# vwxyzjn/cleanrl

Hardware: AMD Instinct MI355X
Metric: env-steps/sec (SPS) PPO Breakout num_envs=1024 @1/2/4/8 MI355X; GAE HBM GB/s (higher is better)
Workload: dtype f32

## Files before the change

cleanrl_amd/build.py:

```python
from __future__ import annotations

import os
import subprocess
import sys
from concurrent.futures import ThreadPoolExecutor

CSRC = os.path.join(os.path.dirname(os.path.abspath(__file__)), "csrc")
LIB = os.path.join(CSRC, "libmi355ppo.so")
SOURCES = ["api.hip", "gae.hip", "distributions.hip", "loss.hip", "obs.hip", "optim.hip", "conv.hip", "convw.hip", "conv1q.hip", "conv1p.hip", "gemmz.hip", "gemmg.hip", "gemmh.hip", "convr.hip", "convrb.hip", "convrs.hip", "convu.hip", "fcw.hip", "heads.hip", "mlp.hip", "synth_env.hip", "dpcomm.hip", "lstm.hip", "trxl_attn.hip", "impala.hip", "pqn.hip", "pqn_lstm.hip", "offpolicy.hip", "sac.hip", "dqn.hip", "dqn_atari.hip", "rainbow.hip", "rainbow_twins.hip", "sac_atari.hip", "sac_atari_twins.hip", "qdagger.hip", "rnd.hip", "ppg.hip", "ppg_twins.hip", "host_twins.hip"]
HEADERS = ["common.h", "catrow.h", "ppo_rows.h", "lstm_rows.h", "trxl_rows.h", "impala_rows.h", "pqn_rows.h", "pqn_lstm_rows.h", "offpolicy_rows.h", "offpolicy_wg.h", "qhead_wg.h", "sac_rows.h", "dqn_rows.h", "dqn_atari_rows.h", "rainbow_rows.h", "sac_atari_rows.h", "qdagger_rows.h", "rnd_rows.h", "ppg_rows.h", "bf16split.h", "f16split.h", "convr_geom.h", "convrb_geom.h", "convrs_geom.h", os.path.join("..", "..", "include", "mi355ppo.h")]
HIPCC = os.environ.get("HIPCC", "/opt/rocm/bin/hipcc")
FLAGS = ["--offload-arch=gfx950", "-O3", "-std=c++20", "-ffp-contract=off", "-fPIC", "-fvisibility=hidden", "-Wall", "-Wno-unused-function"]
EXTRA_FLAGS = {"conv.hip": ["-mllvm", "-pragma-unroll-threshold=1000000"], "gemmz.hip": ["-fno-slp-vectorize"], "gemmg.hip": ["-fno-slp-vectorize"], "gemmh.hip": ["-fno-slp-vectorize", "-mllvm", "-pragma-unroll-threshold=1000000"], "convr.hip": ["-fno-slp-vectorize", "-mllvm", "-pragma-unroll-threshold=1000000"], "convrb.hip": ["-fno-slp-vectorize", "-mllvm", "-pragma-unroll-threshold=1000000"], "convrs.hip": ["-fno-slp-vectorize", "-mllvm", "-pragma-unroll-threshold=1000000"], "convu.hip": ["-fno-slp-vectorize", "-mllvm", "-pragma-unroll-threshold=1000000"], "fcw.hip": ["-fno-slp-vectorize"], "convw.hip": ["-fno-slp-vectorize"], "lstm.hip": ["-fno-slp-vectorize"], "pqn_lstm.hip": ["-fno-slp-vectorize"]}


def _stale(target: str, deps: list[str]) -> bool:
    if not os.path.exists(target):
        return True
    t = os.path.getmtime(target)
    return any(os.path.getmtime(d) > t for d in deps)


def _run(cmd: list[str]) -> None:
    r = subprocess.run(cmd, cwd=CSRC, capture_output=True, text=True)
    if r.returncode != 0:
        raise RuntimeError("command failed: %s\n%s\n%s" % (" ".join(cmd), r.stdout, r.stderr))


def build(force: bool = False, verbose: bool = True) -> str:
    hdrs = [os.path.join(CSRC, h) for h in HEADERS]
    objs, jobs = [], []
    for src in SOURCES:
        obj = os.path.join(CSRC, src.replace(".hip", ".o"))
        objs.append(obj)
        if force or _stale(obj, [os.path.join(CSRC, src)] + hdrs):
            jobs.append([HIPCC] + FLAGS + EXTRA_FLAGS.get(src, []) + ["-c", src, "-o", obj])
    if jobs:
        if verbose:
            print(f"[cleanrl_amd.build] compiling {len(jobs)} HIP source(s) for gfx950", file=sys.stderr)
        with ThreadPoolExecutor(max_workers=min(len(jobs), os.cpu_count() or 1)) as ex:
            list(ex.map(_run, jobs))
    if force or jobs or _stale(LIB, objs):
        _run([HIPCC, "--offload-arch=gfx950", "-shared", "-o", LIB] + objs)
        if verbose:
            print(f"[cleanrl_amd.build] linked {LIB}", file=sys.stderr)
    return LIB


def build_tools(verbose: bool = True) -> str:
    root = os.path.dirname(os.path.dirname(CSRC))
    src = os.path.join(root, "tools", "conv_traffic.cpp")
    exe = os.path.join(root, "tools", "conv_traffic")
    if _stale(exe, [src, LIB, os.path.join(root, "include", "mi355ppo.h")]):
        _run([HIPCC, "--offload-arch=gfx950", "-O2", "-I" + os.path.join(root, "include"), src, "-o", exe, "-L" + CSRC,
              "-lmi355ppo", "-Wl,-rpath,$ORIGIN/../cleanrl_amd/csrc"])
        if verbose:
            print(f"[cleanrl_amd.build] built {exe}", file=sys.stderr)
    fsrc, fexe = os.path.join(root, "tools", "mfma_floor.cpp"), os.path.join(root, "tools", "mfma_floor")
    if os.path.exists(fsrc) and _stale(fexe, [fsrc]):
        _run([HIPCC, "--offload-arch=gfx950", "-O3", fsrc, "-o", fexe])
        if verbose:
            print(f"[cleanrl_amd.build] built {fexe}", file=sys.stderr)
    psrc, pexe = os.path.join(root, "tools", "hbm_probe.cpp"), os.path.join(root, "tools", "hbm_probe")
    if os.path.exists(psrc) and _stale(pexe, [psrc]):
        _run([HIPCC, "--offload-arch=gfx950", "-O3", psrc, "-o", pexe])
        if verbose:
            print(f"[cleanrl_amd.build] built {pexe}", file=sys.stderr)
    dsrc, dexe = os.path.join(root, "tools", "mfma_denorm.cpp"), os.path.join(root, "tools", "mfma_denorm")
    if os.path.exists(dsrc) and _stale(dexe, [dsrc]):
        _run([HIPCC, "--offload-arch=gfx950", "-O2", "-Wno-unused-result", dsrc, "-o", dexe])
        if verbose:
            print(f"[cleanrl_amd.build] built {dexe}", file=sys.stderr)
    return exe


if __name__ == "__main__":
    build(force="--force" in sys.argv)
    build_tools()
```

cleanrl_amd/csrc/common.h:

```cpp
#pragma once
#include <hip/hip_runtime.h>
#include <stdint.h>
#include <stdio.h>
#include <stdarg.h>
#include <stdlib.h>

#include "../../include/mi355ppo.h"

#define MI355_WAVE 64
#ifndef MI355_AUX_WGRAD_LD
#define MI355_AUX_WGRAD_LD 2
#endif
#ifndef MI355_AUX_STREAM_LD
#define MI355_AUX_STREAM_LD 0
#endif
#ifndef MI355_AUX_STREAM_ST
#define MI355_AUX_STREAM_ST 0
#endif
#define MI355_HD __host__ __device__ __forceinline__

namespace mi355ppo {

void set_error(const char* fmt, ...);

int conv1p_launch(const unsigned char* src, const int64_t* inds, const float* dz, float* part_w, float* part_b, int images, int grid,
                  hipStream_t s, const unsigned* dz_amax, float* partial_scale);
bool convw_applies(int64_t images, int layer, bool f16 = false);
int convw_parts(int64_t images, int layer);
int convw_launch(const float* src, const float* dz, float* part_w, float* part_b, int64_t images, int layer, int* nparts, hipStream_t s,
                 const unsigned* dz_amax = nullptr, const unsigned* src_amax = nullptr);

bool convr_on(long long images, long long min_images);
int convr_fwd3(const char* fn, const float* src, unsigned src_bytes, const void* pack, const float* bias, float* dst, unsigned dst_bytes, unsigned* bits,
               long long images, const unsigned* src_amax, unsigned* dst_amax, hipStream_t st);
int convr_fwd2(const char* fn, const float* src, unsigned src_bytes, const void* pack, const float* bias, float* dst, unsigned dst_bytes, unsigned* bits,
               long long images, const unsigned* src_amax, unsigned* dst_amax, hipStream_t st);
int convr_dgrad3(const char* fn, const float* dz, unsigned dz_bytes, const void* pack, const unsigned* bits, float* dsrc, unsigned dsrc_bytes,
                 long long images, const unsigned* dz_amax, unsigned* dsrc_amax, hipStream_t st);
int convr_dgrad2(const char* fn, const float* dz, unsigned dz_bytes, const void* pack, const unsigned* bits, float* dsrc, unsigned dsrc_bytes,
                 long long images, const unsigned* dz_amax, unsigned* dsrc_amax, hipStream_t st);
#ifndef MI355_RING_DMA
#define MI355_RING_DMA 1
#endif
#ifndef MI355_RB_MIN_IMAGES
#define MI355_RB_MIN_IMAGES 3072
#endif
bool convrb_takes(long long images);
int convrb_dgrad2(const char* fn, const float* dz, unsigned dz_bytes, const void* pack, const unsigned* bits, float* dsrc, unsigned dsrc_bytes,
                  long long images, const unsigned* dz_amax, unsigned* dsrc_amax, hipStream_t st);
#ifndef MI355_RS_MIN_IMAGES
#define MI355_RS_MIN_IMAGES 512
#endif
bool convrs_takes(long long images);
int convrs_fwd2(const char* fn, const float* src, unsigned src_bytes, const void* pack, const float* bias, float* dst, unsigned dst_bytes, unsigned* bits,
                long long images, const unsigned* src_amax, unsigned* dst_amax, hipStream_t st);
int convu_max_parts();
bool convu_takes(int64_t images, int layer);
int convu_launch(const float* src, const float* dz, float* part_w, float* part_b, int64_t images, int layer, int* nparts, hipStream_t s,
                 const unsigned* dz_amax, const unsigned* src_amax);
int convu1_launch(const unsigned char* frames, const int64_t* inds, const float* dz, float* part_w, float* part_b, int64_t images, int* nparts,
                  hipStream_t s, const unsigned* dz_amax);
bool gemmg_on(long long rows, long long min_rows);
int gemmg_launch(const char* fn, int epi, const float* A, int lda, const void* pack, const float* bias, const unsigned* bits, float* C, int M, int N,
                 int K, const unsigned* a_amax, unsigned* c_amax, hipStream_t s);
bool gemmh_takes(int M, int N, int K, int lddz);
int gemmh_slabs();
int gemmh_launch(const float* dz, int lddz, const float* a, float* part, int M, int N, int K, const unsigned* dz_amax, const unsigned* a_amax, hipStream_t s);
int z_fc_raw_launch(const char* fn, const float* a, int lda, const void* pack, int M, int N, int K, void* ws, size_t ws_bytes, int* splits,
                    hipStream_t stream, const unsigned* a_amax = nullptr);

inline hipStream_t as_stream(void* s) { return reinterpret_cast<hipStream_t>(s); }

inline int bf16_term_pairs() {
    static const int n = [] {
        const char* e = getenv("MI355PPO_BF16_PAIRS");
        return (e && e[0] == '9') ? 9 : 6;
    }();
    return n;
}

inline bool kernel_switch(const char* name, long long size, long long default_min) {
    const char* e = getenv(name);
    if (!e || !e[0]) return size >= default_min;
    if (e[0] == '0' && !e[1]) return false;
    if (e[0] == 'm' && e[1] == 'i' && e[2] == 'n' && e[3] == ':') return size >= atoll(e + 4);
    return size >= default_min;
}

inline bool aligned(const void* p, size_t a) { return (reinterpret_cast<uintptr_t>(p) % a) == 0; }

inline int check_launch(const char* what) {
    hipError_t e = hipGetLastError();
    if (e != hipSuccess) {
        set_error("%s: %s", what, hipGetErrorString(e));
        return MI355PPO_EHIP;
    }
    return MI355PPO_OK;
}

#define MI355_REQUIRE(cond, code, ...)          \
    do {                                        \
        if (!(cond)) {                          \
            ::mi355ppo::set_error(__VA_ARGS__); \
            return (code);                      \
        }                                       \
    } while (0)

#ifdef __HIPCC__

MI355_HD uint32_t mulhi_u32(uint32_t a, uint32_t b) {
#if defined(__HIP_DEVICE_COMPILE__)
    return __umulhi(a, b);
#else
    return (uint32_t)(((uint64_t)a * (uint64_t)b) >> 32);
#endif
}

struct Philox {
    uint32_t k0, k1;
    MI355_HD Philox(uint64_t seed) : k0((uint32_t)seed), k1((uint32_t)(seed >> 32)) {}
    MI355_HD uint4 operator()(uint64_t ctr_lo, uint64_t ctr_hi) const {
        uint32_t c0 = (uint32_t)ctr_lo, c1 = (uint32_t)(ctr_lo >> 32), c2 = (uint32_t)ctr_hi, c3 = (uint32_t)(ctr_hi >> 32);
        uint32_t a = k0, b = k1;
#pragma unroll
        for (int r = 0; r < 10; ++r) {
            const uint32_t hi0 = mulhi_u32(0xD2511F53u, c0), lo0 = 0xD2511F53u * c0;
            const uint32_t hi1 = mulhi_u32(0xCD9E8D57u, c2), lo1 = 0xCD9E8D57u * c2;
            const uint32_t n0 = hi1 ^ c1 ^ a, n1 = lo1, n2 = hi0 ^ c3 ^ b, n3 = lo0;
            c0 = n0; c1 = n1; c2 = n2; c3 = n3;
            a += 0x9E3779B9u; b += 0xBB67AE85u;
        }
        return make_uint4(c0, c1, c2, c3);
    }
};

MI355_HD float u32_to_unit_open(uint32_t x) {
    return ((float)(x >> 9) + 0.5f) * (1.0f / 8388608.0f);
}


__device__ __forceinline__ float wave_sum(float v) {
#pragma unroll
    for (int off = 32; off > 0; off >>= 1) v += __shfl_xor(v, off, MI355_WAVE);
    return v;
}
__device__ __forceinline__ double wave_sum(double v) {
#pragma unroll
    for (int off = 32; off > 0; off >>= 1) v += __shfl_xor(v, off, MI355_WAVE);
    return v;
}

template <int NWAVES>
__device__ __forceinline__ double block_sum(double v, double* lds) {
    v = wave_sum(v);
    const int lane = threadIdx.x & 63, wave = threadIdx.x >> 6;
    if (lane == 0) lds[wave] = v;
    __syncthreads();
    double r = 0.0;
    if (threadIdx.x == 0) {
#pragma unroll
        for (int w = 0; w < NWAVES; ++w) r += lds[w];
    }
    __syncthreads();
    return r;
}

#endif
}
```

cleanrl_amd/csrc/gemmz.hip:

```cpp
#include "common.h"
#include "conv1q_pack.h"
#include "bf16split.h"
#include "f16split.h"
#include <type_traits>

#pragma clang fp contract(off)

namespace mi355ppo {

typedef float z_f32x16 __attribute__((ext_vector_type(16)));

__device__ __forceinline__ int z_writelane(int w, unsigned x, int l) {
    asm("s_nop 1\n\tv_writelane_b32 %0, %1, %2" : "+v"(w) : "s"(x), "i"(l));
    return w;
}

enum { Z_BIAS_RELU = 0, Z_MASK = 1, Z_MASK_CLS4 = 2, Z_MASKB = 3, Z_MASKB_CLS4 = 4, Z_BIAS_RELU_BITS = 5, Z_RAW = 6 };

__device__ __forceinline__ float z_keep_where(float x, unsigned lo, unsigned hi) {
    const unsigned long long m = ((unsigned long long)hi << 32) | lo;
    float r;
    asm("s_nop 1\n\tv_cndmask_b32_e64 %0, 0, %1, %2" : "=v"(r) : "v"(x), "s"(m));
    return r;
}
// ... 1001 lines not shown
    ZArgs za = zargs(a, (long long)M * lda * 4, lda, pack, bias, nullptr, h, (long long)M * N * 4, N, M, N, K);
    za.a_amax = a_amax; za.c_amax = h_amax;
    if (a_amax && fc_g_takes(M, N, K, false)) {
        rc = gemmg_launch(fn, 0, a, lda, pack, bias, nullptr, h, M, N, K, a_amax, h_amax, as_stream(stream));
        if (rc <= 0) return rc;
    }
    if (M < 16384) return z_launch<ZRowsLinear, 2, 2, 4, Z_BIAS_RELU, true, 2>(za, as_stream(stream), fn);
    return z_launch<ZRowsLinear, 2, 4, 4, Z_BIAS_RELU, true>(za, as_stream(stream), fn);
}

extern "C" MI355PPO_API int mi355ppo_fc_fwd_relu_packed_f32(const float* a, int lda, const void* pack, const float* bias, float* h,
                                                            int M, int N, int K, void* stream) {
    return fc_fwd_impl("mi355ppo_fc_fwd_relu_packed_f32", a, lda, pack, bias, h, M, N, K, nullptr, nullptr, stream);
}

static int fc_fwd_ws_impl(const char* fn, const float* a, int lda, const void* pack, const float* bias, float* h, int M, int N, int K, void* ws,
                          size_t ws_bytes, const unsigned* a_amax, unsigned* h_amax, void* stream) {
    const size_t need = mi355ppo_fc_fwd_workspace_bytes(M, N, K);
    if (need == 0 || !ws || N % 4) return fc_fwd_impl(fn, a, lda, pack, bias, h, M, N, K, a_amax, h_amax, stream);
    MI355_REQUIRE(!h_amax, MI355PPO_EINVAL, "%s: the K-split forward (M=%d) does not record h's maximum (no consumer splits h: pass null)", fn, M);
    int rc = zgemm_check(fn, a, pack, h, M, N, K, lda, N);
    if (rc) return rc;
    MI355_REQUIRE(bias && aligned(bias, 4) && aligned(h, 16) && aligned(ws, 16), MI355PPO_EINVAL, "%s: bias missing, or h / workspace not 16-byte aligned", fn);
    MI355_REQUIRE(ws_bytes >= need, MI355PPO_EINVAL, "%s: workspace of %zu bytes, %zu needed (mi355ppo_fc_fwd_workspace_bytes)", fn, ws_bytes, need);
    ZArgs za = zargs(a, (long long)M * lda * 4, lda, pack, bias, nullptr, static_cast<float*>(ws), (long long)M * N * 4, N, M, N, K);
    za.a_amax = a_amax;
    za.steps_per = zsplit_steps_per(M, N, K);
    const int splits = (K / 16 + za.steps_per - 1) / za.steps_per;
    rc = z_launch<ZRowsLinear, 2, 2, 4, Z_RAW, true, 2>(za, as_stream(stream), fn);
    if (rc) return rc;
    const size_t total4 = (size_t)M * N / 4;
    hipLaunchKernelGGL(zsplit_reduce_kernel, dim3((unsigned)((total4 + 255) / 256)), dim3(256), 0, as_stream(stream),
                       static_cast<const float4*>(ws), splits, total4, bias, N / 4, reinterpret_cast<float4*>(h), total4);
    return check_launch(fn);
}

extern "C" MI355PPO_API int mi355ppo_fc_fwd_relu_packed_ws_f32(const float* a, int lda, const void* pack, const float* bias, float* h,
                                                               int M, int N, int K, void* ws, size_t ws_bytes, void* stream) {
    return fc_fwd_ws_impl("mi355ppo_fc_fwd_relu_packed_ws_f32", a, lda, pack, bias, h, M, N, K, ws, ws_bytes, nullptr, nullptr, stream);
}

namespace mi355ppo {
int z_fc_raw_launch(const char* fn, const float* a, int lda, const void* pack, int M, int N, int K, void* ws, size_t ws_bytes, int* splits,
                    hipStream_t stream, const unsigned* a_amax) {
    const size_t need = mi355ppo_fc_fwd_workspace_bytes(M, N, K);
    MI355_REQUIRE(need > 0 && N % 4 == 0, MI355PPO_EINVAL, "%s: M=%d rows need no K split (use the unfused entry points from 8,192 rows on)", fn, M);
    int rc = zgemm_check(fn, a, pack, static_cast<const float*>(ws), M, N, K, lda, N);
    if (rc) return rc;
    MI355_REQUIRE(ws && aligned(ws, 16) && ws_bytes >= need, MI355PPO_EWORKSPACE, "%s: workspace of %zu bytes, %zu needed (mi355ppo_fc_fwd_workspace_bytes)",
                  fn, ws ? ws_bytes : (size_t)0, need);
    ZArgs za = zargs(a, (long long)M * lda * 4, lda, pack, nullptr, nullptr, static_cast<float*>(ws), (long long)M * N * 4, N, M, N, K);
    za.a_amax = a_amax;
    za.steps_per = zsplit_steps_per(M, N, K);
    *splits = (K / 16 + za.steps_per - 1) / za.steps_per;
    return z_launch<ZRowsLinear, 2, 2, 4, Z_RAW, true, 2>(za, stream, fn);
}
}

static int fc_dgrad_impl(const char* fn, const float* dz, int lddz, const void* pack, const float* act_in, const unsigned* bits, float* da,
                         int M, int N, int K, void* stream, const unsigned* dz_amax = nullptr, unsigned* da_amax = nullptr) {
    int rc = zgemm_check(fn, dz, pack, da, M, N, K, lddz, N);
    if (rc) return rc;
    ZArgs za = zargs(dz, (long long)M * lddz * 4, lddz, pack, nullptr, act_in, da, (long long)M * N * 4, N, M, N, K);
    za.a_amax = dz_amax; za.c_amax = da_amax;
    za.super_rows = 4;
    if (bits) {
        MI355_REQUIRE(N % 32 == 0 && aligned(bits, 4) && aligned(da, 128), MI355PPO_EINVAL, "%s: bit masks need N %% 32 == 0 (N=%d) and da on a 128-byte boundary", fn, N);
        za.bits_in = bits;
        if (dz_amax && fc_g_takes(M, N, K, true)) {
            rc = gemmg_launch(fn, 1, dz, lddz, pack, nullptr, bits, da, M, N, K, dz_amax, da_amax, as_stream(stream));
            if (rc <= 0) return rc;
        }
        return z_launch<ZRowsLinear, 2, 4, 4, Z_MASKB, false>(za, as_stream(stream), fn);
    }
    MI355_REQUIRE(act_in && aligned(act_in, 4) && act_in != da, MI355PPO_EINVAL, "%s: act_in missing, misaligned or aliased with da", fn);
    return z_launch<ZRowsLinear, 2, 4, 4, Z_MASK, false>(za, as_stream(stream), fn);
}

extern "C" MI355PPO_API int mi355ppo_fc_dgrad_mask_packed_f32(const float* dz, int lddz, const void* pack, const float* act_in, float* da,
                                                              int M, int N, int K, void* stream) {
    return fc_dgrad_impl("mi355ppo_fc_dgrad_mask_packed_f32", dz, lddz, pack, act_in, nullptr, da, M, N, K, stream);
}

extern "C" MI355PPO_API int mi355ppo_fc_dgrad_maskbits_packed_f32(const float* dz, int lddz, const void* pack, const uint32_t* mask_bits,
                                                                  float* da, int M, int N, int K, void* stream) {
    const char* fn = "mi355ppo_fc_dgrad_maskbits_packed_f32";
    MI355_REQUIRE(mask_bits, MI355PPO_EINVAL, "%s: null pointer", fn);
    return fc_dgrad_impl(fn, dz, lddz, pack, nullptr, mask_bits, da, M, N, K, stream);
}

static bool conv_r_takes(long long images, int layer, bool dgrad) {
    return convr_on(images, dgrad && layer == 2 ? 512 : 1);
}

static int conv_fwd_packed_impl(const char* fn, const float* src, const void* pack, const float* bias, float* dst, unsigned* bits,
                                int64_t images, int layer, void* stream, const unsigned* src_amax = nullptr, unsigned* dst_amax = nullptr) {
    MI355_REQUIRE(src && pack && bias && dst, MI355PPO_EINVAL, "%s: null pointer", fn);
    MI355_REQUIRE(layer == 2 || layer == 3, MI355PPO_EINVAL, "%s: layer=%d must be 2 or 3", fn, layer);
    MI355_REQUIRE(images > 0, MI355PPO_EINVAL, "%s: images=%lld must be positive", fn, (long long)images);
    MI355_REQUIRE(aligned(src, 16) && aligned(pack, 16) && aligned(dst, 128) && aligned(bias, 4) && aligned(bits, 4), MI355PPO_EALIGN,
                  "%s: src / pack must be 16-byte aligned, dst 128-byte aligned", fn);
    const long long srcb = (long long)images * (layer == 2 ? 20 * 20 * 32 : 9 * 9 * 64) * 4;
    MI355_REQUIRE(srcb < (1LL << 32) - 8192, MI355PPO_EINVAL, "%s: the source (%lld bytes) must stay below 4 GiB (32-bit buffer offsets)", fn, srcb);
    hipStream_t st = as_stream(stream);
    const bool small = !bits && images < 768;
    if (layer == 2) {
        if (src_amax && conv_r_takes(images, 2, false)) {
            if (convrs_takes(images)) return convrs_fwd2(fn, src, (unsigned)srcb, pack, bias, dst, (unsigned)((long long)images * 81 * 64 * 4), bits, images, src_amax, dst_amax, st);
            return convr_fwd2(fn, src, (unsigned)srcb, pack, bias, dst, (unsigned)((long long)images * 81 * 64 * 4), bits, images, src_amax, dst_amax, st);
        }
        ZArgs za = zargs(src, srcb, 0, pack, bias, nullptr, dst, (long long)images * 81 * 64 * 4, 64, (long long)images * 81, 64, ZConv2::K);
        za.bits_out = bits;
        za.a_amax = src_amax; za.c_amax = dst_amax;
        if (small) return z_launch<ZConv2, 1, 2, 4, Z_BIAS_RELU, false, 2>(za, st, fn);
        if (bits) return z_blds(images) ? z_launch<ZConv2, 2, 2, 4, Z_BIAS_RELU_BITS, false, 2, true>(za, st, fn) : z_launch<ZConv2, 2, 2, 4, Z_BIAS_RELU_BITS, false, 2>(za, st, fn);
        return z_blds(images) ? z_launch<ZConv2, 2, 2, 4, Z_BIAS_RELU, false, 2, true>(za, st, fn) : z_launch<ZConv2, 2, 2, 4, Z_BIAS_RELU, false, 2>(za, st, fn);
    }
    if (src_amax && conv_r_takes(images, 3, false))
        return convr_fwd3(fn, src, (unsigned)srcb, pack, bias, dst, (unsigned)((long long)images * 49 * 64 * 4), bits, images, src_amax, dst_amax, st);
    ZArgs za = zargs(src, srcb, 0, pack, bias, nullptr, dst, (long long)images * 49 * 64 * 4, 64, (long long)images * 49, 64, ZConv3::K);
    za.bits_out = bits;
    za.a_amax = src_amax; za.c_amax = dst_amax;
    if (small) return z_launch<ZConv3, 1, 2, 4, Z_BIAS_RELU, false, 2>(za, st, fn);
    if (bits) return z_blds(images) ? z_launch<ZConv3, 2, 2, 4, Z_BIAS_RELU_BITS, false, 2, true>(za, st, fn) : z_launch<ZConv3, 2, 2, 4, Z_BIAS_RELU_BITS, false, 2>(za, st, fn);
    return z_blds(images) ? z_launch<ZConv3, 2, 2, 4, Z_BIAS_RELU, false, 2, true>(za, st, fn) : z_launch<ZConv3, 2, 2, 4, Z_BIAS_RELU, false, 2>(za, st, fn);
}

extern "C" MI355PPO_API int mi355ppo_cnn_conv_fwd_packed_f32(const float* src, const void* pack, const float* bias, float* dst,
                                                             int64_t images, int layer, void* stream) {
    return conv_fwd_packed_impl("mi355ppo_cnn_conv_fwd_packed_f32", src, pack, bias, dst, nullptr, images, layer, stream);
}

extern "C" MI355PPO_API int mi355ppo_cnn_conv_fwd_packed_bits_f32(const float* src, const void* pack, const float* bias, float* dst,
                                                                  uint32_t* mask_bits, int64_t images, int layer, void* stream) {
    const char* fn = "mi355ppo_cnn_conv_fwd_packed_bits_f32";
    MI355_REQUIRE(mask_bits, MI355PPO_EINVAL, "%s: null pointer", fn);
    return conv_fwd_packed_impl(fn, src, pack, bias, dst, mask_bits, images, layer, stream);
}

static int conv_dgrad_packed_impl(const char* fn, const float* dz, const void* pack, const float* act_in, const unsigned* bits, float* dsrc,
                                  int64_t images, int layer, void* stream, const unsigned* dz_amax = nullptr, unsigned* dsrc_amax = nullptr) {
    MI355_REQUIRE(dz && pack && (act_in || bits) && dsrc, MI355PPO_EINVAL, "%s: null pointer", fn);
    MI355_REQUIRE(layer == 2 || layer == 3, MI355PPO_EINVAL, "%s: layer=%d must be 2 or 3", fn, layer);
    MI355_REQUIRE(images > 0, MI355PPO_EINVAL, "%s: images=%lld must be positive", fn, (long long)images);
    MI355_REQUIRE(aligned(dz, 16) && aligned(pack, 16) && aligned(dsrc, 128) && aligned(act_in, 16) && aligned(bits, 4), MI355PPO_EALIGN,
                  "%s: dz / pack / act_in must be 16-byte aligned, dsrc 128-byte aligned", fn);
    MI355_REQUIRE(act_in != dsrc, MI355PPO_EINVAL, "%s: act_in must not alias dsrc", fn);
    const long long srcb = (long long)images * (layer == 2 ? 9 * 9 * 64 : 7 * 7 * 64) * 4;
    const long long dstb = (long long)images * (layer == 2 ? 20 * 20 * 32 : 9 * 9 * 64) * 4;
    MI355_REQUIRE(srcb < (1LL << 32) - 8192 && dstb < (1LL << 32) - 8192, MI355PPO_EINVAL,
                  "%s: dz (%lld bytes) and dsrc (%lld bytes) must stay below 4 GiB (32-bit buffer offsets)", fn, srcb, dstb);
    hipStream_t st = as_stream(stream);
    if (layer == 3) {
        if (dz_amax && bits && conv_r_takes(images, 3, true)) return convr_dgrad3(fn, dz, (unsigned)srcb, pack, bits, dsrc, (unsigned)dstb, images, dz_amax, dsrc_amax, st);
        ZArgs za = zargs(dz, srcb, 0, pack, nullptr, act_in, dsrc, (long long)images * 81 * 64 * 4, 64, (long long)images * 81, 64, ZDgrad3::K, images);
        za.bits_in = bits;
        za.a_amax = dz_amax; za.c_amax = dsrc_amax;
        if (bits) return z_blds(images) ? z_launch<ZDgrad3, 2, 2, 4, Z_MASKB, false, 2, true>(za, st, fn) : z_launch<ZDgrad3, 2, 2, 4, Z_MASKB, false, 2>(za, st, fn);
        return z_blds(images) ? z_launch<ZDgrad3, 2, 2, 4, Z_MASK, false, 2, true>(za, st, fn) : z_launch<ZDgrad3, 2, 2, 4, Z_MASK, false, 2>(za, st, fn);
    }
    if (dz_amax && bits && conv_r_takes(images, 2, true)) return convr_dgrad2(fn, dz, (unsigned)srcb, pack, bits, dsrc, (unsigned)dstb, images, dz_amax, dsrc_amax, st);
    ZArgs za = zargs(dz, srcb, 0, pack, nullptr, act_in, dsrc, (long long)images * 400 * 32 * 4, 0, (long long)images * 100, 128, ZDgrad2::K, images);
    za.bits_in = bits;
    za.a_amax = dz_amax; za.c_amax = dsrc_amax;
    if (bits) return z_blds(images) ? z_launch<ZDgrad2, 2, 2, 4, Z_MASKB_CLS4, false, 2, true>(za, st, fn) : z_launch<ZDgrad2, 2, 2, 4, Z_MASKB_CLS4, false, 2>(za, st, fn);
    return z_blds(images) ? z_launch<ZDgrad2, 2, 2, 4, Z_MASK_CLS4, false, 2, true>(za, st, fn) : z_launch<ZDgrad2, 2, 2, 4, Z_MASK_CLS4, false, 2>(za, st, fn);
}

extern "C" MI355PPO_API int mi355ppo_cnn_conv_dgrad_packed_f32(const float* dz, const void* pack, const float* act_in, float* dsrc,
                                                               int64_t images, int layer, void* stream) {
    const char* fn = "mi355ppo_cnn_conv_dgrad_packed_f32";
    MI355_REQUIRE(act_in, MI355PPO_EINVAL, "%s: null pointer", fn);
    return conv_dgrad_packed_impl(fn, dz, pack, act_in, nullptr, dsrc, images, layer, stream);
}

extern "C" MI355PPO_API int mi355ppo_cnn_conv_dgrad_packed_bits_f32(const float* dz, const void* pack, const uint32_t* mask_bits, float* dsrc,
                                                                    int64_t images, int layer, void* stream) {
    const char* fn = "mi355ppo_cnn_conv_dgrad_packed_bits_f32";
    MI355_REQUIRE(mask_bits, MI355PPO_EINVAL, "%s: null pointer", fn);
    return conv_dgrad_packed_impl(fn, dz, pack, nullptr, mask_bits, dsrc, images, layer, stream);
}

extern "C" MI355PPO_API int mi355ppo_cnn_conv_packed_kernel_f16x2(int64_t images, int layer, int dgrad) {
    if (!(images > 0 && (layer == 2 || layer == 3) && conv_r_takes(images, layer, dgrad != 0))) return 'Z';
    return (layer == 2 && dgrad != 0 && convrb_takes(images)) ? 'B' : 'R';
}

extern "C" MI355PPO_API size_t mi355ppo_fc_pack_f16x2_bytes(int N, int K) {
    if (N <= 0 || K <= 0 || K % 16) return 0;
    return (size_t)kF16PackHeader + (size_t)(K / 16) * (size_t)((N + 31) / 32) * 2048;
}

extern "C" MI355PPO_API int mi355ppo_absmax_f32(const float* x, int64_t n, uint32_t* amax, void* stream) {
    const char* fn = "mi355ppo_absmax_f32";
    MI355_REQUIRE(x && amax, MI355PPO_EINVAL, "%s: null pointer", fn);
    MI355_REQUIRE(n > 0, MI355PPO_EINVAL, "%s: n=%lld must be positive", fn, (long long)n);
    MI355_REQUIRE(aligned(x, 4) && aligned(amax, 64), MI355PPO_EALIGN, "%s: the amax record must be 64-byte aligned", fn);
    ZAbsmax3 m;
    m.x[0] = x; m.n[0] = n; m.x[1] = m.x[2] = x; m.n[1] = m.n[2] = 0;
    long long blocks = (n / 4 + 255) / 256;
    if (blocks < 1) blocks = 1;
    if (blocks > 2048) blocks = 2048;
    hipLaunchKernelGGL(zabsmax_kernel, dim3((unsigned)blocks), dim3(256), 0, as_stream(stream), m, amax, (int)blocks);
    return check_launch(fn);
}

extern "C" MI355PPO_API int mi355ppo_fc_pack_f16x2_f32(const float* B, int ldb, int N, int K, const uint32_t* b_amax, void* pack, void* stream) {
    const char* fn = "mi355ppo_fc_pack_f16x2_f32";
    MI355_REQUIRE(B && pack && b_amax, MI355PPO_EINVAL, "%s: null pointer", fn);
    MI355_REQUIRE(N > 0 && K > 0 && K % 16 == 0 && ldb >= K, MI355PPO_EINVAL, "%s: N=%d K=%d ldb=%d (K a positive multiple of 16, ldb >= K)", fn, N, K, ldb);
    MI355_REQUIRE(aligned(B, 4) && aligned(pack, 16) && aligned(b_amax, 64), MI355PPO_EALIGN, "%s: misaligned pointer (pack: 16 bytes, record: 64)", fn);
    const long long total = (long long)(K / 16) * ((N + 31) / 32) * 512;
    hipLaunchKernelGGL(zpack_h_kernel, dim3((unsigned)((total + 255) / 256)), dim3(256), 0, as_stream(stream), B, ldb, N, K, b_amax,
                       static_cast<unsigned char*>(pack));
    return check_launch(fn);
}

extern "C" MI355PPO_API int mi355ppo_fc_fwd_relu_packed_f16x2_f32(const float* a, int lda, const void* pack, const float* bias, float* h, int M,
                                                                  int N, int K, void* ws, size_t ws_bytes, const uint32_t* a_amax,
                                                                  uint32_t* h_amax, void* stream) {
    const char* fn = "mi355ppo_fc_fwd_relu_packed_f16x2_f32";
    MI355_REQUIRE(a_amax && aligned(a_amax, 64) && aligned(h_amax, 64), MI355PPO_EINVAL, "%s: a's amax record missing, or a record not 64-byte aligned", fn);
    return fc_fwd_ws_impl(fn, a, lda, pack, bias, h, M, N, K, ws, ws_bytes, a_amax, h_amax, stream);
}

extern "C" MI355PPO_API int mi355ppo_fc_dgrad_packed_f16x2_f32(const float* dz, int lddz, const void* pack, const float* act_in,
                                                               const uint32_t* mask_bits, float* da, int M, int N, int K, const uint32_t* dz_amax,
                                                               uint32_t* da_amax, void* stream) {
    const char* fn = "mi355ppo_fc_dgrad_packed_f16x2_f32";
    MI355_REQUIRE(dz_amax && aligned(dz_amax, 64) && aligned(da_amax, 64), MI355PPO_EINVAL, "%s: dz's amax record missing, or a record not 64-byte aligned", fn);
    MI355_REQUIRE(act_in || mask_bits, MI355PPO_EINVAL, "%s: neither act_in nor mask_bits", fn);
    return fc_dgrad_impl(fn, dz, lddz, pack, mask_bits ? nullptr : act_in, mask_bits, da, M, N, K, stream, dz_amax, da_amax);
}

extern "C" MI355PPO_API int mi355ppo_cnn_conv_fwd_packed_f16x2_f32(const float* src, const void* pack, const float* bias, float* dst,
                                                                   uint32_t* mask_bits, int64_t images, int layer, const uint32_t* src_amax,
                                                                   uint32_t* dst_amax, void* stream) {
    const char* fn = "mi355ppo_cnn_conv_fwd_packed_f16x2_f32";
    MI355_REQUIRE(src_amax && aligned(src_amax, 64) && aligned(dst_amax, 64), MI355PPO_EINVAL, "%s: src's amax record missing, or a record not 64-byte aligned", fn);
    return conv_fwd_packed_impl(fn, src, pack, bias, dst, mask_bits, images, layer, stream, src_amax, dst_amax);
}

extern "C" MI355PPO_API int mi355ppo_cnn_conv_dgrad_packed_f16x2_f32(const float* dz, const void* pack, const float* act_in,
                                                                     const uint32_t* mask_bits, float* dsrc, int64_t images, int layer,
                                                                     const uint32_t* dz_amax, uint32_t* dsrc_amax, void* stream) {
    const char* fn = "mi355ppo_cnn_conv_dgrad_packed_f16x2_f32";
    MI355_REQUIRE(dz_amax && aligned(dz_amax, 64) && aligned(dsrc_amax, 64), MI355PPO_EINVAL, "%s: dz's amax record missing, or a record not 64-byte aligned", fn);
    return conv_dgrad_packed_impl(fn, dz, pack, mask_bits ? nullptr : act_in, mask_bits, dsrc, images, layer, stream, dz_amax, dsrc_amax);
}
```

Baseline: 1.386 million.

## Add persistent LDS-resident conv3 dgrad kernel with DMA weight ring

Adds a new persistent kernel for the layer-3 conv data-gradient (7x7x64 to 9x9x64) that stages each group of 7 images in LDS as split f16 hi/lo pairs. It streams packed weights through a double-buffered ring filled by LDS-DMA buffer loads and prefetches the next group's input during the k-loop. Output rows are packed into tiles by a compile-time table grouped by border class, so MFMA tiles skip inactive taps. It is selected over the existing convr path when images reach 4096, and it adds a large amount of hand-scheduled code whose correctness depends on the vmcnt accounting.

```diff
diff --git a/cleanrl_amd/build.py b/cleanrl_amd/build.py
--- a/cleanrl_amd/build.py
+++ b/cleanrl_amd/build.py
@@ -7,11 +7,11 @@
 
 CSRC = os.path.join(os.path.dirname(os.path.abspath(__file__)), "csrc")
 LIB = os.path.join(CSRC, "libmi355ppo.so")
-SOURCES = ["api.hip", "gae.hip", "distributions.hip", "loss.hip", "obs.hip", "optim.hip", "conv.hip", "convw.hip", "conv1q.hip", "conv1p.hip", "gemmz.hip", "gemmg.hip", "gemmh.hip", "convr.hip", "convrb.hip", "convrs.hip", "convu.hip", "fcw.hip", "heads.hip", "mlp.hip", "synth_env.hip", "dpcomm.hip", "lstm.hip", "trxl_attn.hip", "impala.hip", "pqn.hip", "pqn_lstm.hip", "offpolicy.hip", "sac.hip", "dqn.hip", "dqn_atari.hip", "rainbow.hip", "rainbow_twins.hip", "sac_atari.hip", "sac_atari_twins.hip", "qdagger.hip", "rnd.hip", "ppg.hip", "ppg_twins.hip", "host_twins.hip"]
-HEADERS = ["common.h", "catrow.h", "ppo_rows.h", "lstm_rows.h", "trxl_rows.h", "impala_rows.h", "pqn_rows.h", "pqn_lstm_rows.h", "offpolicy_rows.h", "offpolicy_wg.h", "qhead_wg.h", "sac_rows.h", "dqn_rows.h", "dqn_atari_rows.h", "rainbow_rows.h", "sac_atari_rows.h", "qdagger_rows.h", "rnd_rows.h", "ppg_rows.h", "bf16split.h", "f16split.h", "convr_geom.h", "convrb_geom.h", "convrs_geom.h", os.path.join("..", "..", "include", "mi355ppo.h")]
+SOURCES = ["api.hip", "gae.hip", "distributions.hip", "loss.hip", "obs.hip", "optim.hip", "conv.hip", "convw.hip", "conv1q.hip", "conv1p.hip", "gemmz.hip", "gemmg.hip", "gemmh.hip", "convr.hip", "convrb.hip", "convrs.hip", "convrv.hip", "convu.hip", "fcw.hip", "heads.hip", "mlp.hip", "synth_env.hip", "dpcomm.hip", "lstm.hip", "trxl_attn.hip", "impala.hip", "pqn.hip", "pqn_lstm.hip", "offpolicy.hip", "sac.hip", "dqn.hip", "dqn_atari.hip", "rainbow.hip", "rainbow_twins.hip", "sac_atari.hip", "sac_atari_twins.hip", "qdagger.hip", "rnd.hip", "ppg.hip", "ppg_twins.hip", "host_twins.hip"]
+HEADERS = ["common.h", "catrow.h", "ppo_rows.h", "lstm_rows.h", "trxl_rows.h", "impala_rows.h", "pqn_rows.h", "pqn_lstm_rows.h", "offpolicy_rows.h", "offpolicy_wg.h", "qhead_wg.h", "sac_rows.h", "dqn_rows.h", "dqn_atari_rows.h", "rainbow_rows.h", "sac_atari_rows.h", "qdagger_rows.h", "rnd_rows.h", "ppg_rows.h", "bf16split.h", "f16split.h", "convr_geom.h", "convrb_geom.h", "convrs_geom.h", "convrv_geom.h", os.path.join("..", "..", "include", "mi355ppo.h")]
 HIPCC = os.environ.get("HIPCC", "/opt/rocm/bin/hipcc")
 FLAGS = ["--offload-arch=gfx950", "-O3", "-std=c++20", "-ffp-contract=off", "-fPIC", "-fvisibility=hidden", "-Wall", "-Wno-unused-function"]
-EXTRA_FLAGS = {"conv.hip": ["-mllvm", "-pragma-unroll-threshold=1000000"], "gemmz.hip": ["-fno-slp-vectorize"], "gemmg.hip": ["-fno-slp-vectorize"], "gemmh.hip": ["-fno-slp-vectorize", "-mllvm", "-pragma-unroll-threshold=1000000"], "convr.hip": ["-fno-slp-vectorize", "-mllvm", "-pragma-unroll-threshold=1000000"], "convrb.hip": ["-fno-slp-vectorize", "-mllvm", "-pragma-unroll-threshold=1000000"], "convrs.hip": ["-fno-slp-vectorize", "-mllvm", "-pragma-unroll-threshold=1000000"], "convu.hip": ["-fno-slp-vectorize", "-mllvm", "-pragma-unroll-threshold=1000000"], "fcw.hip": ["-fno-slp-vectorize"], "convw.hip": ["-fno-slp-vectorize"], "lstm.hip": ["-fno-slp-vectorize"], "pqn_lstm.hip": ["-fno-slp-vectorize"]}
+EXTRA_FLAGS = {"conv.hip": ["-mllvm", "-pragma-unroll-threshold=1000000"], "gemmz.hip": ["-fno-slp-vectorize"], "gemmg.hip": ["-fno-slp-vectorize"], "gemmh.hip": ["-fno-slp-vectorize", "-mllvm", "-pragma-unroll-threshold=1000000"], "convr.hip": ["-fno-slp-vectorize", "-mllvm", "-pragma-unroll-threshold=1000000"], "convrb.hip": ["-fno-slp-vectorize", "-mllvm", "-pragma-unroll-threshold=1000000"], "convrs.hip": ["-fno-slp-vectorize", "-mllvm", "-pragma-unroll-threshold=1000000"], "convrv.hip": ["-fno-slp-vectorize", "-mllvm", "-pragma-unroll-threshold=1000000"], "convu.hip": ["-fno-slp-vectorize", "-mllvm", "-pragma-unroll-threshold=1000000"], "fcw.hip": ["-fno-slp-vectorize"], "convw.hip": ["-fno-slp-vectorize"], "lstm.hip": ["-fno-slp-vectorize"], "pqn_lstm.hip": ["-fno-slp-vectorize"]}
 
 
 def _stale(target: str, deps: list[str]) -> bool:
diff --git a/cleanrl_amd/csrc/common.h b/cleanrl_amd/csrc/common.h
--- a/cleanrl_amd/csrc/common.h
+++ b/cleanrl_amd/csrc/common.h
@@ -54,6 +54,12 @@
 bool convrs_takes(long long images);
 int convrs_fwd2(const char* fn, const float* src, unsigned src_bytes, const void* pack, const float* bias, float* dst, unsigned dst_bytes, unsigned* bits,
                 long long images, const unsigned* src_amax, unsigned* dst_amax, hipStream_t st);
+#ifndef MI355_RV_MIN_IMAGES
+#define MI355_RV_MIN_IMAGES 4096
+#endif
+bool convrv_takes(long long images);
+int convrv_dgrad3(const char* fn, const float* dz, unsigned dz_bytes, const void* pack, const unsigned* bits, float* dsrc, unsigned dsrc_bytes,
+                  long long images, const unsigned* dz_amax, unsigned* dsrc_amax, hipStream_t st);
 int convu_max_parts();
 bool convu_takes(int64_t images, int layer);
 int convu_launch(const float* src, const float* dz, float* part_w, float* part_b, int64_t images, int layer, int* nparts, hipStream_t s,
diff --git a/cleanrl_amd/csrc/convrv.hip b/cleanrl_amd/csrc/convrv.hip
--- /dev/null
+++ b/cleanrl_amd/csrc/convrv.hip
@@ -0,0 +1,304 @@
+#include "common.h"
+#include "f16split.h"
+#include "convrv_geom.h"
+
+#pragma clang fp contract(off)
+
+namespace mi355ppo {
+
+typedef float rv_f32x16 __attribute__((ext_vector_type(16)));
+
+constexpr unsigned kRVOob = 0xFFFFF000u;
+constexpr int kRVRsrcWord3 = 0x00020000;
+constexpr int kRVWaitVm0 = 0x0F70;
+
+__device__ __forceinline__ float rv_keep_where(float x, unsigned lo, unsigned hi) {
+    const unsigned long long m = ((unsigned long long)hi << 32) | lo;
+    float r;
+    asm("s_nop 1\n\tv_cndmask_b32_e64 %0, 0, %1, %2" : "=v"(r) : "v"(x), "s"(m));
+    return r;
+}
+
+__device__ __forceinline__ void rv_dma16(__amdgpu_buffer_rsrc_t rsrc, unsigned char* dst, unsigned voff, int soff) {
+    __builtin_amdgcn_raw_ptr_buffer_load_lds(rsrc, (__attribute__((address_space(3))) void*)dst, 16, voff, soff, 0, 0);
+}
+
+struct RVArgs {
+    const float* A;
+    unsigned a_bytes;
+    const unsigned char* pack;
+    const unsigned* bits_in;
+    float* C;
+    unsigned c_bytes;
+    long long images;
+    int groups;
+    int grid;
+    const unsigned* a_amax;
+    unsigned* c_amax;
+};
+
+template <int XC>
+__device__ __forceinline__ void rv_wave(const RVArgs& a, unsigned char* const lds, const int tid, const int wave) {
+    using RG = RVGeom;
+    constexpr int NT = RG::NT, NW = RG::NW, NI = RG::NI, THREADS = RG::THREADS, SS = RG::SS, NSLOT = RG::NSLOT;
+    constexpr int MT = 4 + XC, NWM = (MT + 1) / 2;
+    constexpr int kPieces = SS * NT * 2;
+    constexpr int kShare = kPieces / NW;
+    static_assert(kPieces % NW == 0 && MI355_RING_DMA, "whole pieces per wave; the ring by LDS-DMA only");
+    unsigned char* const ring = lds + RG::ABYTES;
+    unsigned* const rofft = reinterpret_cast<unsigned*>(lds + RG::ABYTES + 2 * RG::SLOTB);
+    const int lane = tid & 63, li = lane & 31, lh = lane >> 5;
+    const int simd = wave & 3, jc = wave >> 2;
+    auto tile_of = [&](int i) __attribute__((always_inline)) -> int {
+        return i < 2 ? 2 * simd + i : (i == 2 ? 10 + simd : (i == 3 ? 14 + simd : 8 + (simd >> 1)));
+    };
+
+    const int ea = f16_scale_exp(amax_load(a.a_amax, lane));
+    const int eb = f16_scale_exp(*reinterpret_cast<const unsigned*>(a.pack));
+    const float sa = f16_pow2(ea), un = f16_unscale(ea, eb);
+
+    constexpr RVRowTable table{};
+    auto origin = [&](int tile, int ty) __attribute__((always_inline)) -> unsigned {
+        const int id = table.src[tile * 32 + li];
+        const int gi = id / RG::OP, p = id - gi * RG::OP, y = p / RG::OW, x = p - y * RG::OW;
+        return (unsigned)(rv_origin(gi, y, x, ty) * RG::PIX + 16 * lh);
+    };
+    unsigned winc[2 + XC], winb[3];
+    winc[0] = origin(tile_of(0), 0);
+    winc[1] = origin(tile_of(1), 0);
+    if constexpr (XC) winc[2] = origin(tile_of(4), 0);
+    const bool eb_pair = simd >= 2;
+    winb[0] = origin(10 + simd, 0);
+    winb[1] = origin(eb_pair ? 14 + simd : 10 + simd, 1);
+    winb[2] = origin(14 + simd, 2);
+
+    const __amdgpu_buffer_rsrc_t rsrc_a = __builtin_amdgcn_make_buffer_rsrc(const_cast<float*>(a.A), 0, (int)a.a_bytes, kRVRsrcWord3);
+    unsigned udst[(NI + 1) / 2];
+#pragma unroll
+    for (int it = 0; it < NI; ++it) {
+        const int u = it * THREADS + tid;
+        const int pix = u / RG::UPP, c4 = u - pix * RG::UPP, img = pix / (RG::IH * RG::IW), q = pix - img * (RG::IH * RG::IW), qy = q / RG::IW, qx = q - qy * RG::IW;
+        const unsigned d = u < RG::UNITS ? (unsigned)(RG::rec(img, qy, qx) * RG::PIX + c4 * 8) >> 3 : 0xffffu;
+        udst[it >> 1] = (it & 1) ? (udst[it >> 1] | (d << 16)) : d;
+    }
+    static_assert(rv_pre_lo(RG::KSTEPS) == NI, "the next group's source is requested inside one k-loop");
+    s_u32x4 pre[NI];
+    auto prefetch = [&](int grp, int it0, int n) __attribute__((always_inline)) {
+        const bool any = grp < a.groups;
+        const unsigned base = (unsigned)grp * (unsigned)(RG::UNITS * 16);
+#pragma unroll
+        for (int it = it0; it < it0 + n && it < NI; ++it) {
+            const int u = it * THREADS + tid;
+            pre[it] = __builtin_bit_cast(s_u32x4, __builtin_amdgcn_raw_buffer_load_b128(rsrc_a, (any && u < RG::UNITS) ? base + (unsigned)u * 16u : kRVOob, 0, MI355_AUX_STREAM_LD));
+        }
+    };
+    auto fill = [&]() __attribute__((always_inline)) {
+#pragma unroll
+        for (int it = 0; it < NI; ++it) {
+            unsigned hi[2], lo[2];
+            f16_split4(pre[it], sa, hi, lo);
+            if ((it & 1) == 0) asm volatile("" : "+v"(udst[it >> 1]));
+            const unsigned d = (it & 1) ? udst[it >> 1] >> 16 : udst[it >> 1] & 0xffffu;
+            if ((it + 1) * THREADS <= RG::UNITS || d != 0xffffu) {
+                *reinterpret_cast<uint2*>(lds + 8u * d) = make_uint2(hi[0], hi[1]);
+                *reinterpret_cast<uint2*>(lds + 8u * d + RG::LO) = make_uint2(lo[0], lo[1]);
+            }
+        }
+    };
+
+    const unsigned col_off = (unsigned)(jc * 32 * 4);
+    auto rsrc_c_of = [&](int g, unsigned gbase) __attribute__((always_inline)) {
+        const bool ok = g >= 0 && g < a.groups;
+        return __builtin_amdgcn_make_buffer_rsrc(reinterpret_cast<unsigned char*>(a.C) + (ok ? gbase : 0u), 0, ok ? (int)(a.c_bytes - gbase) : 0, kRVRsrcWord3);
+    };
+    auto rsrc_b_of = [&](int g) __attribute__((always_inline)) {
+        return __builtin_amdgcn_make_buffer_rsrc(const_cast<unsigned*>(a.bits_in), 0, (g >= 0 && g < a.groups) ? (int)(a.c_bytes >> 5) : 0, kRVRsrcWord3);
+    };
+    float cmax = 0.0f;
+
+    const __amdgpu_buffer_rsrc_t rsrc_p = __builtin_amdgcn_make_buffer_rsrc(const_cast<unsigned char*>(a.pack), 0, kF16PackHeader + RG::KSTEPS * RG::STEPB, kRVRsrcWord3);
+    const unsigned lane16 = 16u * (unsigned)lane;
+    int gpar = 0;
+    unsigned rbuf[2] = {(unsigned)(RG::ABYTES + 16 * lane + jc * 2048), (unsigned)(RG::ABYTES + RG::SLOTB + 16 * lane + jc * 2048)};
+    auto dma_slot = [&](int slot) __attribute__((always_inline)) {
+#pragma unroll
+        for (int u = 0; u < kShare; ++u) {
+            const int x = wave * kShare + u, h = x / (NT * 2), jt = x - h * (NT * 2);
+            rv_dma16(rsrc_p, ring + ((slot & 1) ^ gpar) * RG::SLOTB + x * 1024, lane16, kF16PackHeader + (SS * (slot % NSLOT) + h) * RG::STEPB + jt * 1024);
+        }
+    };
+    auto dma_wait = [&](int slot) __attribute__((always_inline)) {
+        const int n = rv_dma_younger(slot);
+#define RV_VMCNT_CASE(k) if (n == k) asm volatile("s_waitcnt vmcnt(" #k ")" ::: "memory");
+        RV_VMCNT_CASE(1) RV_VMCNT_CASE(2) RV_VMCNT_CASE(3) RV_VMCNT_CASE(4) RV_VMCNT_CASE(5) RV_VMCNT_CASE(6)
+#undef RV_VMCNT_CASE
+        if (n < 1 || n > 6) asm volatile("s_waitcnt vmcnt(0)" ::: "memory");
+    };
+    auto ring_barrier = [&]() __attribute__((always_inline)) {
+        asm volatile("s_waitcnt lgkmcnt(0)" ::: "memory");
+        __builtin_amdgcn_s_barrier();
+    };
+
+    rv_f32x16 acc[MT];
+    unsigned wm[NWM];
+    s_u32x4 pa[4][2], wb[2][2];
+    auto read_a = [&](int pos, unsigned w, int off) __attribute__((always_inline)) {
+        pa[pos][0] = *reinterpret_cast<const s_u32x4*>(lds + w + off);
+        pa[pos][1] = *reinterpret_cast<const s_u32x4*>(lds + w + off + RG::LO);
+    };
+    auto read_c = [&](int pos, int i, int v) __attribute__((always_inline)) { read_a(pos, winc[i], rv_tapoff_c(v)); };
+    auto read_bd = [&](int pos, int v) __attribute__((always_inline)) { read_a(pos, winb[v / RG::SPR], rv_tapoff_b(v)); };
+    auto read_b = [&](int par, int v) __attribute__((always_inline)) {
+        const int h = v % SS;
+#pragma unroll
+        for (int t = 0; t < 2; ++t) wb[par][t] = *reinterpret_cast<const s_u32x4*>(lds + rbuf[(v / SS) & 1] + (h * NT * 2 + t) * 1024);
+    };
+    unsigned mword[NWM];
+#pragma unroll
+    for (int k = 0; k < NWM; ++k) {
+        const int t = (2 * k + 1 < MT && lh) ? tile_of(2 * k + 1) : tile_of(2 * k);
+        mword[k] = (unsigned)((t * 2 + ((li >> 2) & 1)) * 16 + (li & 3) + 4 * (li >> 3));
+    }
+    auto load_masks = [&](unsigned gbase, const __amdgpu_buffer_rsrc_t rb) __attribute__((always_inline)) {
+#pragma unroll
+        for (int k = 0; k < NWM; ++k) {
+            const bool have = 2 * k + 1 < MT || lh == 0;
+            const unsigned ro = rofft[mword[k]];
+            wm[k] = __builtin_amdgcn_raw_buffer_load_b32(rb, have ? (gbase + ro) >> 5 : kRVOob, 0, 0);
+        }
+    };
+    auto mfma3 = [&](int q, int t, int p, int pi, bool z) __attribute__((always_inline)) {
+        if (pi == 0 && z) {
+#pragma unroll
+            for (int e = 0; e < 16; ++e) acc[t][e] = 0.0f;
+        }
+        acc[t] = __builtin_amdgcn_mfma_f32_32x32x16_f16(__builtin_bit_cast(s_f16x8, pa[p][pi == 2 ? 1 : 0]), __builtin_bit_cast(s_f16x8, wb[q][pi == 1 ? 1 : 0]), acc[t], 0, 0, 0);
+    };
+    auto pair = [&](int q, int t0, int p0, bool z0, int t1, int p1, bool z1) __attribute__((always_inline)) {
+#pragma unroll
+        for (int pi = 0; pi < 3; ++pi) {
+            mfma3(q, t0, p0, pi, z0);
+            if (t1 >= 0) mfma3(q, t1, p1, pi, z1);
+        }
+    };
+
+    auto group = [&](int grp) __attribute__((always_inline)) {
+        const unsigned gbase = (unsigned)grp * (unsigned)RG::GROUPC + col_off;
+        const __amdgpu_buffer_rsrc_t rb_cur = rsrc_b_of(grp);
+        ring_barrier();
+        fill();
+        __builtin_amdgcn_sched_barrier(0);
+        ring_barrier();
+#pragma unroll
+        for (int e = 0; e < 16; ++e) acc[3][e] = 0.0f;
+        read_b(0, 0);
+        read_c(0, 0, 0); read_c(1, 1, 0); read_bd(2, 0);
+        if constexpr (XC) read_c(3, 2, 0);
+#pragma unroll
+        for (int v = 0; v < RG::KSTEPS; ++v) {
+            const int q = v & 1, slot = v / SS, h = v % SS;
+            if (v + 1 < RG::KSTEPS) {
+                if (h == SS - 1) {
+                    dma_wait(slot);
+                    ring_barrier();
+                }
+                read_b(q ^ 1, v + 1);
+            }
+            if (h == 0) {
+                dma_slot(slot + 1);
+                __builtin_amdgcn_sched_barrier(0);
+            }
+            if (rv_pre_lo(v + 1) > rv_pre_lo(v)) prefetch(grp + a.grid, rv_pre_lo(v), rv_pre_lo(v + 1) - rv_pre_lo(v));
+            if (v == RG::KSTEPS - 3) load_masks(gbase, rb_cur);
+            if (h == 0 && (slot == 3 || slot == 6) && eb_pair) {
+                const rv_f32x16 t = acc[2];
+                acc[2] = acc[3];
+                acc[3] = t;
+            }
+            __builtin_amdgcn_sched_barrier(0);
+            pair(q, 0, 0, v == 0, 1, 1, v == 0);
+            __builtin_amdgcn_sched_barrier(0);
+            if (v + 1 < RG::KSTEPS) { read_c(0, 0, v + 1); read_c(1, 1, v + 1); }
+            __builtin_amdgcn_sched_barrier(0);
+            if constexpr (XC) pair(q, 2 + (slot >= 6 ? 1 : 0), 2, v == 0 && slot < 6, 4, 3, v == 0);
+            else pair(q, 2 + (slot >= 6 ? 1 : 0), 2, v == 0 && slot < 6, -1, 0, false);
+            __builtin_amdgcn_sched_barrier(0);
+            if (v + 1 < RG::KSTEPS) {
+                read_bd(2, v + 1);
+                if constexpr (XC) read_c(3, 2, v + 1);
+            }
+            __builtin_amdgcn_sched_barrier(0);
+        }
+        __builtin_amdgcn_s_waitcnt(kRVWaitVm0);
+        __builtin_amdgcn_sched_barrier(0);
+        const __amdgpu_buffer_rsrc_t rc = rsrc_c_of(grp, gbase);
+#pragma unroll
+        for (int i = 0; i < MT; ++i) {
+            const unsigned* const rt = rofft + (tile_of(i) * 2 + lh) * 16;
+            unsigned ro[16];
+#pragma unroll
+            for (int e4 = 0; e4 < 4; ++e4) {
+                const s_u32x4 w = *reinterpret_cast<const s_u32x4*>(rt + 4 * e4);
+                ro[4 * e4] = w[0]; ro[4 * e4 + 1] = w[1]; ro[4 * e4 + 2] = w[2]; ro[4 * e4 + 3] = w[3];
+            }
+#pragma unroll
+            for (int e = 0; e < 16; ++e) {
+                const int wr = 32 * i + (e & 3) + 8 * (e >> 2);
+                const unsigned lo = (unsigned)__builtin_amdgcn_readlane((int)wm[wr >> 6], wr & 63);
+                const unsigned hi = (unsigned)__builtin_amdgcn_readlane((int)wm[(wr + 4) >> 6], (wr + 4) & 63);
+                const float v = rv_keep_where(acc[i][e] * un, lo, hi);
+                cmax = __builtin_fmaxf(cmax, __builtin_fabsf(v));
+                __builtin_amdgcn_raw_buffer_store_b32(__float_as_uint(v), rc, ro[e] + 4u * (unsigned)li, 0, MI355_AUX_STREAM_ST);
+            }
+            __builtin_amdgcn_sched_barrier(0);
+        }
+        gpar ^= 1;
+        const unsigned t = rbuf[0];
+        rbuf[0] = rbuf[1];
+        rbuf[1] = t;
+    };
+
+    int grp = blockIdx.x;
+    if (grp < a.groups) {
+        prefetch(grp, 0, NI);
+        dma_slot(0);
+        __builtin_amdgcn_s_waitcnt(kRVWaitVm0);
+    }
+    for (; grp < a.groups; grp += a.grid) group(grp);
+    if (a.c_amax) amax_commit(a.c_amax, __float_as_uint(cmax), blockIdx.x * NW + (unsigned)wave, lane);
+}
+
+__global__ __launch_bounds__(RVGeom::THREADS) __attribute__((amdgpu_waves_per_eu(2, 2))) void rv_kernel(RVArgs a) {
+    using RG = RVGeom;
+    __shared__ __attribute__((aligned(16))) unsigned char lds[RG::LDSB];
+    const int tid = threadIdx.x, wave = __builtin_amdgcn_readfirstlane(tid >> 6);
+    for (int o = tid * 16; o < RG::ABYTES; o += RG::THREADS * 16) *reinterpret_cast<s_u32x4*>(lds + o) = (s_u32x4){0u, 0u, 0u, 0u};
+    constexpr RVRowTable table{};
+    unsigned* const rofft = reinterpret_cast<unsigned*>(lds + RG::ABYTES + 2 * RG::SLOTB);
+    for (int w = tid; w < RG::TILES * 32; w += RG::THREADS) {
+        const int t = w >> 5, h = (w >> 4) & 1, e = w & 15;
+        rofft[w] = (unsigned)table.src[t * 32 + (e & 3) + 8 * (e >> 2) + 4 * h] * (unsigned)(32 * RG::NT * 4);
+    }
+    if (RG::extra(wave)) rv_wave<1>(a, lds, tid, wave);
+    else rv_wave<0>(a, lds, tid, wave);
+}
+
+bool convrv_takes(long long images) { return kernel_switch("MI355PPO_CONV_RV", images, MI355_RV_MIN_IMAGES); }
+
+int convrv_dgrad3(const char* fn, const float* dz, unsigned dz_bytes, const void* pack, const unsigned* bits, float* dsrc, unsigned dsrc_bytes,
+                  long long images, const unsigned* dz_amax, unsigned* dsrc_amax, hipStream_t st) {
+    RVArgs a{};
+    a.A = dz; a.a_bytes = dz_bytes; a.pack = static_cast<const unsigned char*>(pack); a.bits_in = bits; a.C = dsrc; a.c_bytes = dsrc_bytes;
+    a.images = images; a.a_amax = dz_amax; a.c_amax = dsrc_amax;
+    a.groups = (int)((images + RVGeom::G - 1) / RVGeom::G);
+    int dev = 0, cus = 0;
+    if (hipGetDevice(&dev) != hipSuccess || hipDeviceGetAttribute(&cus, hipDeviceAttributeMultiprocessorCount, dev) != hipSuccess || cus <= 0) {
+        (void)hipGetLastError();
+        cus = 256;
+    }
+    a.grid = a.groups < cus ? a.groups : cus;
+    hipLaunchKernelGGL(rv_kernel, dim3((unsigned)a.grid), dim3(RVGeom::THREADS), 0, st, a);
+    return check_launch(fn);
+}
+
+}
diff --git a/cleanrl_amd/csrc/convrv_geom.h b/cleanrl_amd/csrc/convrv_geom.h
--- /dev/null
+++ b/cleanrl_amd/csrc/convrv_geom.h
@@ -0,0 +1,107 @@
+#pragma once
+
+#if defined(__HIPCC__)
+#define RV_GEOM_FN __device__ __forceinline__ constexpr
+#else
+#define RV_GEOM_FN inline constexpr
+#endif
+
+namespace mi355ppo {
+
+struct RVGeom {
+    static constexpr int IH = 7, IW = 7, IC = 64, OH = 9, OW = 9, OP = OH * OW, KH = 3, KW = 3, HL = 2;
+    static constexpr int G = 7, NW = 8, NT = 2, TILES = 18, CT = 10;
+    static constexpr int RP = 9, IPIX = IH * RP, RECS = G * IPIX + 2;
+    static constexpr int PIX = 4 * IC + 16, LO = 2 * IC, C16 = IC / 16;
+    static constexpr int KSTEPS = KH * KW * C16, SS = 4, NSLOT = KSTEPS / SS, SPR = KW * C16;
+    static constexpr int ABYTES = RECS * PIX;
+    static constexpr int STEPB = NT * 2048, SLOTB = SS * STEPB;
+    static constexpr int ROWS = G * OP, SLOTS = 32 * TILES;
+    static constexpr int UPP = IC / 4, UNITS = G * IH * IW * UPP, THREADS = 64 * NW, NI = (UNITS + THREADS - 1) / THREADS;
+    static constexpr int ROFFB = TILES * 2 * 16 * 4;
+    static constexpr int LDSB = ABYTES + 2 * SLOTB + ROFFB;
+    static constexpr int GROUPC = G * OP * 32 * NT * 4;
+    static constexpr int rec(int gi, int qy, int qx) { return gi * IPIX + qy * RP + HL + qx; }
+    static constexpr int cls_of(int y) { return y == 0 ? 0 : y == 1 ? 1 : y <= 6 ? 2 : y == 7 ? 3 : 4; }
+    static constexpr int ty_first(int cls) { return cls == 0 ? 2 : cls == 1 ? 1 : 0; }
+    static constexpr int ty_last(int cls) { return cls == 3 ? 1 : cls == 4 ? 0 : 2; }
+    static constexpr int tile_cls(int t) { return t < CT ? 2 : t < 12 ? 3 : t < 14 ? 4 : t < 16 ? 0 : 1; }
+    static constexpr int slot_first(int t) { return 3 * ty_first(tile_cls(t)); }
+    static constexpr int slot_last(int t) { return 3 * ty_last(tile_cls(t)) + 2; }
+    static constexpr bool active(int t, int slot) { return slot >= slot_first(t) && slot <= slot_last(t); }
+    static constexpr int simd_of(int w) { return w & 3; }
+    static constexpr int col_of(int w) { return w >> 2; }
+    static constexpr bool extra(int w) { return (simd_of(w) & 1) == col_of(w); }
+    static constexpr int ntiles(int w) { return extra(w) ? 5 : 4; }
+    static constexpr int wave_tile(int w, int i) { return i < 2 ? 2 * simd_of(w) + i : i == 2 ? 10 + simd_of(w) : i == 3 ? 14 + simd_of(w) : 8 + (simd_of(w) >> 1); }
+    static constexpr int border_tile(int w, int ty) { return ty <= ty_last(tile_cls(10 + simd_of(w))) ? 10 + simd_of(w) : 14 + simd_of(w); }
+};
+
+static_assert(RVGeom::LDSB <= 160 * 1024 && (RVGeom::PIX / 16) % 2 == 1 && RVGeom::ROWS <= RVGeom::SLOTS && RVGeom::KSTEPS % RVGeom::SS == 0, "LDS, odd pitch, row slots, whole ring slots");
+static_assert(RVGeom::ABYTES / 8 < 0xffff, "two 16-bit record offsets per register");
+
+RV_GEOM_FN int rv_tapoff_c(int ks) {
+    const int ty = ks / RVGeom::SPR, us = ks - ty * RVGeom::SPR, tx = us / RVGeom::C16, chunk = us - tx * RVGeom::C16;
+    return (ty * RVGeom::RP + tx) * RVGeom::PIX + chunk * 32;
+}
+RV_GEOM_FN int rv_tapoff_b(int ks) {
+    const int us = ks % RVGeom::SPR, tx = us / RVGeom::C16, chunk = us - tx * RVGeom::C16;
+    return tx * RVGeom::PIX + chunk * 32;
+}
+RV_GEOM_FN int rv_origin(int gi, int y, int x, int ty) { return RVGeom::rec(gi, y + ty - RVGeom::HL, x - RVGeom::HL); }
+
+struct RVRowTable {
+    short row[RVGeom::SLOTS], src[RVGeom::SLOTS];
+    static constexpr bool first_set(int l) { return l < 4 || (l >= 12 && l < 16) || (l >= 20 && l < 28); }
+    constexpr RVRowTable() : row{}, src{} {
+        using RG = RVGeom;
+        constexpr int NSET = RG::SLOTS / 16;
+        int fill[NSET] = {};
+        bool has[NSET][16] = {};
+        int slot_of[NSET][16] = {};
+        for (int s = 0; s < NSET; ++s) {
+            int k = 0;
+            for (int l = 0; l < 32; ++l)
+                if (first_set(l) == ((s & 1) == 0)) slot_of[s][k++] = (s >> 1) * 32 + l;
+        }
+        for (int i = 0; i < RG::SLOTS; ++i) row[i] = -1;
+        bool done[RG::ROWS] = {};
+        for (int cls = 0; cls < 5; ++cls) {
+            int sets[2 * RG::CT] = {}, ns = 0;
+            for (int t = 0; t < RG::TILES; ++t)
+                if (RG::tile_cls(t) == cls) { sets[ns++] = 2 * t; sets[ns++] = 2 * t + 1; }
+            int next = 0;
+            for (int pass = 0; pass < 2; ++pass)
+                for (int r = 0; r < RG::ROWS; ++r) {
+                    const int gi = r / RG::OP, p = r - gi * RG::OP, y = p / RG::OW, x = p - y * RG::OW;
+                    if (RG::cls_of(y) != cls || done[r]) continue;
+                    const int c = rv_origin(gi, y, x, RG::ty_first(cls)) & 15;
+                    bool placed = false;
+                    for (int t = 0; t < ns && !placed; ++t) {
+                        const int k = (next + t) % ns, s = sets[k];
+                        if (fill[s] < 16 && (pass == 1 || !has[s][c])) {
+                            row[slot_of[s][fill[s]++]] = (short)r;
+                            has[s][c] = true;
+                            placed = true;
+                            done[r] = true;
+                            next = k + 1;
+                        }
+                    }
+                }
+        }
+        for (int s = 0; s < NSET; ++s) {
+            int have = -1;
+            for (int k = 0; k < 16; ++k)
+                if (row[slot_of[s][k]] >= 0) { have = row[slot_of[s][k]]; break; }
+            for (int k = 0; k < 16; ++k) src[slot_of[s][k]] = row[slot_of[s][k]] >= 0 ? row[slot_of[s][k]] : (short)have;
+        }
+    }
+};
+
+RV_GEOM_FN int rv_pre_lo(int v) {
+    const int n = (v - 1) * 2;
+    return v < 1 ? 0 : (n > RVGeom::NI ? RVGeom::NI : n);
+}
+RV_GEOM_FN int rv_dma_younger(int slot) { return rv_pre_lo(RVGeom::SS * slot + RVGeom::SS - 1) - rv_pre_lo(RVGeom::SS * slot); }
+
+}
diff --git a/cleanrl_amd/csrc/gemmz.hip b/cleanrl_amd/csrc/gemmz.hip
--- a/cleanrl_amd/csrc/gemmz.hip
+++ b/cleanrl_amd/csrc/gemmz.hip
@@ -1177,7 +1177,10 @@
                   "%s: dz (%lld bytes) and dsrc (%lld bytes) must stay below 4 GiB (32-bit buffer offsets)", fn, srcb, dstb);
     hipStream_t st = as_stream(stream);
     if (layer == 3) {
-        if (dz_amax && bits && conv_r_takes(images, 3, true)) return convr_dgrad3(fn, dz, (unsigned)srcb, pack, bits, dsrc, (unsigned)dstb, images, dz_amax, dsrc_amax, st);
+        if (dz_amax && bits && conv_r_takes(images, 3, true)) {
+            if (convrv_takes(images)) return convrv_dgrad3(fn, dz, (unsigned)srcb, pack, bits, dsrc, (unsigned)dstb, images, dz_amax, dsrc_amax, st);
+            return convr_dgrad3(fn, dz, (unsigned)srcb, pack, bits, dsrc, (unsigned)dstb, images, dz_amax, dsrc_amax, st);
+        }
         ZArgs za = zargs(dz, srcb, 0, pack, nullptr, act_in, dsrc, (long long)images * 81 * 64 * 4, 64, (long long)images * 81, 64, ZDgrad3::K, images);
         za.bits_in = bits;
         za.a_amax = dz_amax; za.c_amax = dsrc_amax;
```

Measured after the change: 1.404 million, median of 6. 1.01x the previous value.
